# NikolasMarkou/blind_image_denoising

Measured on AMD Instinct MI355X. Metric: denoised images/sec (256x256x3) + MAE vs ref, resnet_1x18, higher is better.
Workload: dtype f16x2 split (hi+lo, fp32 accumulate)

## Files before the change

blind_image_denoising_amd/_native.py:

```python
import ctypes as C
import os
import pathlib

_HERE = pathlib.Path(__file__).resolve().parent
LIB_PATH = pathlib.Path(os.environ.get("BFCNN_HIP_LIB", _HERE / "lib" / "libbfcnn_hip.so"))

BF_OK, BF_EINVAL, BF_EUNSUPPORTED, BF_EWORKSPACE, BF_EHIP = 0, -1, -2, -3, -4
BF_ACT_LINEAR, BF_ACT_RELU, BF_ACT_LEAKY_RELU = 0, 1, 2
BF_REG_NONE, BF_REG_L1, BF_REG_L2 = 0, 1, 2
BF_MODE_INFERENCE, BF_MODE_TRAIN = 0, 1
BF_DTYPE_U8, BF_DTYPE_F32 = 0, 1
BF_LOSS_COUNT = 8
(BF_LOSS_TOTAL, BF_LOSS_DENOISER_TOTAL, BF_LOSS_MAE, BF_LOSS_MSE, BF_LOSS_SSIM,
 BF_LOSS_REGULARIZATION, BF_LOSS_MODEL_TOTAL, BF_LOSS_GRAD_NORM) = range(8)
EPI_RELU, EPI_AFFINE, EPI_RES, EPI_MASK, EPI_STATS, EPI_BNBWD = 1, 2, 4, 8, 16, 32


class ResnetDesc(C.Structure):
    _fields_ = [(n, C.c_int32) for n in (
        "struct_size", "in_channels", "filters", "kernel_size", "no_layers", "block_convs",
        "block_kernel", "activation", "base_activation", "use_bn", "head_filters",
        "head_activation", "out_channels", "denormalize", "reg_base", "reg_block", "reg_head")] + \
        [(n, C.c_float) for n in ("v_min", "v_max", "bn_eps", "bn_momentum", "leaky_alpha")]

# ... 135 lines not shown
    "bf_op_relu_shift_bwd": (_I, [_P, _I, _F, _P, _P, _I, _P]),
    "bf_op_normalize": (_I, [_P, _P, _I64, _F, _F, _I, _P]),
    "bf_op_channel_repeat": (_I, [_P, _P, _I64, _I, _I, _P]),
    "bf_op_channel_group_sum": (_I, [_P, _P, _I64, _I, _I, _P]),
    "bf_op_group_kernel": (_I, [_P, _P, _I, _I, _I, _I, _P]),
    "bf_op_flip_hw": (_I, [_P, _P, _I, _I, _P]),
    "bf_op_transpose2d": (_I, [_P, _P, _I, _I, _P]),
    "bf_comm_unique_id": (_I, [C.c_char_p]),
    "bf_comm_init_rank": (_I, [C.POINTER(_P), _I, _I, C.c_char_p]),
    "bf_comm_destroy": (_I, [_P]),
    "bf_allreduce_grads": (_I, [_P, _P, _I64, _P, _P]),
    "bf_comm_last_error": (C.c_char_p, []),
    "bf_op_channel_multiplier": (_I, [_P, _P, _I, _P]),
    "bf_op_prune_tensors": (_I, [_P, _I64, _P, _I, _I, _F, _F, _F, C.c_uint64, _P, _P, _P]),
    "bf_op_count_below": (_I, [_P, _I64, _P, _I, _F, _P, _P]),
    "bf_op_dihedral_stack_u8": (_I, [_P, _P, _P, _I, _I, _I, _I, _I, _P]),
    "bf_op_dihedral_merge": (_I, [_P, _P, _P, _I, _I, _I, _I, _I, _I, _P]),
    "bf_op_risk_probe_u8": (_I, [_P, _P, _I, _I, _I, _I, _I, _I, C.c_uint64, _P]),
    "bf_op_risk_sums_scratch_bytes": (_I64, [_I, _I, _I, _I, _I]),
    "bf_op_risk_sums": (_I, [_P, _P, _I, _I, _I, _I, _I, _I, C.c_uint64, _P, _I64, _P, _P]),
    "bf_op_risk_sums_affine_scratch_bytes": (_I64, [_I, _I, _I, _I, _I]),
    "bf_op_risk_sums_affine": (_I, [_P, _P, _I, _I, _I, _I, _I, _I, C.c_uint64, _P, _I64, _P, _P]),
    "bf_op_neighbor_pairs": (_I, [_P, _I, _P, _F, _P, _P, _I, _I, _I, _I, C.c_uint64, _P]),
    "bf_set_option": (_I, [_P, C.c_char_p, _I]),
    "bf_get_timing": (_I, [_P, C.POINTER(C.c_float), C.POINTER(C.c_int)]),
    "bf_get_block_kernel": (C.c_char_p, [_P, C.POINTER(C.c_int)]),
    "bf_get_train_kernels": (C.c_char_p, [_P]),
    "bf_debug_conv3x3": (_I, [_P, _P, _P, _P, _P, _P, _P, _P, _P, _I, _I, _I, _I, _I, _P]),
    "bf_debug_conv3x3_grid": (_I, [_I, _I, _I]),
    "bf_debug_h3_weight_scale": (_F, [_F]),
    "bf_debug_fused_block": (_I, [_P, _P, _P, _P, _P, _P, _P, _I, _I, _I, _I, _P]),
    "bf_debug_fused_block_h3_scratch_floats": (_I64, [_I, _I, _I]),
    "bf_debug_fused_block_h3": (_I, [_P, _P, _P, _P, _P, _P, _P, _I, _I, _I, _I, _P]),
    "bf_debug_fused_block2_h3_scratch_floats": (_I64, [_I, _I, _I]),
    "bf_debug_fused_block2_h3": (_I, [_P, _P, _P, _P, _P, _P, _I, _I, _I, _I, _I, _P]),
    "bf_debug_set_h3_variant": (_I, [_I]),
    "bf_debug_set_upsample_band": (_I, [_I]),
    "bf_debug_conv3x3_h3_scratch_floats": (_I64, []),
    "bf_debug_conv3x3_h3": (_I, [_P, _P, _P, _P, _P, _P, _P, _I, _I, _I, _I, _I, _P]),
    "bf_debug_wgrad_partial_floats": (_I64, [_I, _I, _I]),
    "bf_debug_wgrad3x3": (_I, [_P, _P, _P, _P, _I, _I, _I, _P]),
    "bf_debug_wgrad3x3_h3": (_I, [_P, _P, _P, _P, _I, _I, _I, _P]),
    "bf_debug_fwd_block_h3t_scratch_floats": (_I64, [_I, _I, _I]),
    "bf_debug_fwd_block_h3t": (_I, [_P, _P, _P, _P, _P, _P, _P, _P, _P, _P, _P, _I, _I, _I, _I, _I, _P]),
    "bf_debug_bwd_block_h3t_scratch_floats": (_I64, [_I, _I, _I]),
    "bf_debug_bwd_block_h3t": (_I, [_P, _P, _P, _P, _P, _P, _P, _P, _P, _P, _P, _P, _I, _I, _I, _I, _I, _P]),
    "bf_debug_conv3x3_h3_pre": (_I, [_P, _P, _P, _P, _P, _P, _P, _P, _I, _I, _I, _I, _I, _P]),
    "bf_debug_bwd3x3_h3_scratch_floats": (_I64, [_I, _I, _I]),
    "bf_debug_bwd3x3_h3_grid": (_I, [_I, _I, _I]),
    "bf_debug_bwd3x3_h3_grid_ex": (_I, [_I, _I, _I, _I]),
    "bf_debug_bwd3x3_h3": (_I, [_P, _P, _P, _P, _P, _P, _P, _P, _P, _P, _P, _I, _I, _I, _I, _I, _I, _P]),
    "bf_debug_forward_plan": (_I, [_P, _I, _I, _I, _I, C.c_char_p, _I]),
    "bf_debug_base_path": (_I, [_P, _I, _I, _I, _I, _I]),
    "bf_debug_mfma_probe": (_I, [_P, _P, _P, _P]),
}

BF_STATUS_BYTES = 2048
BF_STATUS_F16_RANGE = 1

_lib = None


class StreamArg(C.c_void_p):
    _bf_device = None


def _device_guard(fn):
    def call(*args):
        for a in args:
            dev = getattr(a, "_bf_device", None)
            if dev is not None:
                import torch
                if torch.cuda.current_device() != dev:
                    with torch.cuda.device(dev):
                        return fn(*args)
                break
        return fn(*args)
    call.raw = fn
    call.__name__ = getattr(fn, "__name__", "bf_call")
    return call


class _Library:

    def __init__(self, handle):
        self._handle = handle

    def __getattr__(self, name):
        return getattr(self._handle, name)


def lib():
    global _lib
    if _lib is None:
        if not LIB_PATH.exists():
            raise ImportError(
                f"{LIB_PATH} is missing: the gfx950 HIP library has not been built "
                f"(run blind_image_denoising_amd/csrc/build.sh). There is no CPU fallback.")
        handle = C.CDLL(str(LIB_PATH), mode=getattr(os, "RTLD_NOW", 2))
        wrapped = _Library(handle)
        for name, (res, args) in SIGNATURES.items():
            fn = getattr(handle, name)
            fn.restype = res
            fn.argtypes = args
            setattr(wrapped, name, _device_guard(fn))
        if handle.bf_abi_version() != 1:
# ... 53 lines not shown
```

blind_image_denoising_amd/csrc/bf_common.h:

```cpp
#pragma once
#include <hip/hip_runtime.h>
#include <stdint.h>
#include <stddef.h>
#include "../../include/bfcnn_hip.h"
#include "../../include/bfcnn_hip_debug.h"

typedef float f32x4 __attribute__((ext_vector_type(4)));

__device__ __forceinline__ f32x4 bf_acc_ready(f32x4 acc)
{
    asm volatile("s_nop 7" : "+v"(acc));
    return acc;
}


#include <mutex>
#include <unordered_set>
inline hipError_t bf_set_max_lds(const void* kernel, int bytes)
{
    static std::mutex mu;
    static std::unordered_set<uint64_t> done;
    int dev = 0;
    hipError_t e = hipGetDevice(&dev);
    if (e != hipSuccess) return e;
// ... 98 lines not shown
    int act1_relu;
    const void* zeros;
    void* dump;
    unsigned long long* dbg;
    const float* head_wh;
    void* head_out;
    int head_u8, Ho, Wo, denormalize;
    float v_min, v_max;
    int* status;
    int compact = 0;
};
struct H3Request {
    int B, H, W;
    int variant;
    bool head;
    bool compact;
};
enum class H3Kernel { Tiles32, Tiles16, FullRow };
struct H3Choice {
    H3Kernel kernel;
    bool bottom_up;
};
H3Choice   bf_select_fused_block_h3(const H3Request& r);
hipError_t bf_launch_fused_block_h3_as(const FusedH3Args& a, H3Kernel k, hipStream_t s);
hipError_t bf_launch_fused_block_h3(const FusedH3Args& a, hipStream_t s);
bool       bf_fused_block_h3_use_pairs(const H3Request& r);
const char* bf_fused_block_h3_kernel_name(H3Kernel k);
const char* bf_fused_block_kernel_name();
void       bf_set_h3_variant(int v);
hipError_t bf_launch_fused_block_h3v(const FusedH3Args& a, hipStream_t s);
bool       bf_fused_block_h3v_supports(int H, int W);
struct FusedH3WArgs {
    const void* in;
    void* out;
    const void* w1r[2];
    const void* w2r[2];
    const float* aux[2];
    int B, H, W;
    int nstrips, tiles_y, ntiles, rows_per_tile;
    int reverse_tiles;
    int act1_relu;
    const void* zeros;
    unsigned long long* dbg;
    const float* head_wh;
    void* head_out;
    int head_u8, Ho, Wo, denormalize;
    float v_min, v_max;
    int* status;
    const void* base_u8;
    const float* base_w;
    int Hs, Ws, base_relu;
};
hipError_t bf_launch_fused_block2_h3w(const FusedH3WArgs& a, hipStream_t s);
bool       bf_fused_block2_h3w_supports(int H, int W);
hipError_t bf_launch_pack_h3(const float* params, const float* state, int64_t p_blocks, int64_t p_stride, float* dst,
                             int64_t d_stride, int layers, int use_bn, float eps, const float* ext_scale,
                             const float* ext_shift, hipStream_t s);
#define BF_H3_TRAIN_PACK_FLOATS (BF_H3R_WPACK_FLOATS + 64)
#define BF_TRAIN_PACK_STRIDE BF_H3_TRAIN_PACK_FLOATS
hipError_t bf_launch_conv3x3_h3(const ConvArgs& a, int epi, hipStream_t s);
hipError_t bf_launch_wgrad3x3_h3(const float* x, const float* dy, float* partial, float* dw, int B, int H, int W, hipStream_t s);

struct BwdH3Args {
    const float* x;
    const float* g;
    const float* c;
    const float* coef;
    const float* wpack;
    float* out;
    const float* res;
    const float* bnc;
    float* wpartial;
    float* stats;
    int B, H, W, reverse;
    int reserved[4];
    int tiles_x, tiles_y, ntiles;
};
struct FwdBlockH3Args {
    const float* x;
    const float* pre_c;
    const float* pre_scale; const float* pre_shift;
    float* a_out;
    float* t_out;
    float* c_out;
    const float* wpack0;
    const float* wpack1;
    float* stats;
    int B, H, W, reverse, act_relu;
    int tiles_y, ntiles, rows_per_tile;
    const float* fin_partial;
    int fin_nblk;
    double fin_count;
    const float* fin_gamma;
    float *fin_mm, *fin_mv;
    float fin_eps, fin_momentum;
    float* fin_scale;
    float* fin_meaninv;
};
bool       bf_fwd_block_h3t_supports(int H, int W);
int        bf_fwd_block_h3t_grid(int B, int H, int W);
hipError_t bf_launch_fwd_block_h3t(const FwdBlockH3Args& a, hipStream_t s);
struct BwdBlockH3Args {
    const float* a;
    const float* g;
    const float* c;
    const float* coef;
// ... 106 lines not shown
```

blind_image_denoising_amd/csrc/debug_entry.hip:

```cpp
#include "bf_common.h"
#include "h3_weights.h"
#include <cstring>

extern "C" int bf_debug_conv3x3(const float* in, const float* w_hwio, float* out, const float* scale, const float* shift,
                                const float* res, const float* mask, float* stats, float* wpack_scratch, int B, int H, int W,
                                int epi, int transpose_flip, void* stream)
{
    hipStream_t s = (hipStream_t)stream;
    if (bf_launch_pack_conv(w_hwio, wpack_scratch, transpose_flip, s) != hipSuccess) return BF_EHIP;
    ConvArgs ca;
    memset(&ca, 0, sizeof(ca));
    ca.in = in; ca.out = out; ca.wpack = wpack_scratch; ca.scale = scale; ca.shift = shift; ca.res = res; ca.mask = mask;
    ca.stats = stats; ca.B = B; ca.H = H; ca.W = W;
    return bf_launch_conv3x3_c16(ca, epi, s) == hipSuccess ? BF_OK : BF_EHIP;
}

static unsigned long long* g_fused_dbg = nullptr;
extern "C" int bf_debug_set_fused_dbg(void* buf) { g_fused_dbg = (unsigned long long*)buf; return BF_OK; }

extern "C" int bf_debug_conv3x3_grid(int B, int H, int W) { return bf_conv3x3_c16_grid(B, H, W); }

extern "C" int bf_debug_fused_block(const float* in, const float* w1_hwio, const float* w2_hwio, const float* scale,
                                    const float* shift, float* out, float* wpack_scratch, int B, int H, int W, int act1_relu,
                                    void* stream)
// ... 30 lines not shown
    if (hipMemcpyAsync(params, w1_hwio, 2304 * 4, hipMemcpyDeviceToDevice, s) != hipSuccess) return BF_EHIP;
    if (hipMemcpyAsync(params + 2304, w2_hwio, 2304 * 4, hipMemcpyDeviceToDevice, s) != hipSuccess) return BF_EHIP;
    if (bf_launch_zero(zeros, 64, s) != hipSuccess) return BF_EHIP;
    if (bf_launch_pack_h3(params, state, 0, 4608 + 16, pk, BF_H3_BLOCK_FLOATS, 1, 0, 0.f, scale, shift, s) != hipSuccess) return BF_EHIP;
    if (bf_launch_h3_from_f32(in, xa, B, H, W, s) != hipSuccess) return BF_EHIP;
    FusedH3Args fa;
    fa.in = xa; fa.out = ya; fa.aux = pk;
    fa.w1r = fa.aux + 64; fa.w2r = fa.aux + 64 + BF_H3R_WPACK_FLOATS;
    fa.B = B; fa.H = H; fa.W = W; fa.tiles_x = fa.tiles_y = fa.ntiles = 0; fa.rows_per_tile = 0; fa.variant = -1; fa.reverse_tiles = 0; fa.act1_relu = act1_relu;
    fa.zeros = zeros; fa.dump = dump; fa.dbg = g_fused_dbg;
    fa.head_wh = nullptr; fa.head_out = nullptr; fa.head_u8 = 0; fa.Ho = fa.Wo = 0; fa.denormalize = 0; fa.v_min = fa.v_max = 0.f;
    fa.status = nullptr;
    if (bf_launch_fused_block_h3(fa, s) != hipSuccess) return BF_EHIP;
    return bf_launch_h3_to_f32(ya, out, B, H, W, s) == hipSuccess ? BF_OK : BF_EHIP;
}

extern "C" int64_t bf_debug_fused_block2_h3_scratch_floats(int B, int H, int W)
{
    return 2 * (int64_t)B * H * W * 16 + 2 * (int64_t)BF_H3_BLOCK_FLOATS + 2 * (4608 + 16) + 32 + 64;
}

extern "C" int bf_debug_fused_block2_h3(const float* in, const float* w_hwio, const float* scale, const float* shift, float* out,
                                        float* scratch, int B, int H, int W, int act1_relu, int reverse, void* stream)
{
    hipStream_t s = (hipStream_t)stream;
    if (!in || !w_hwio || !scale || !shift || !out || !scratch || B <= 0 || H <= 0 || W <= 0) return BF_EINVAL;
    const int64_t act = (int64_t)B * H * W * 16;
    float* xa = scratch;
    float* ya = scratch + act;
    float* pk = ya + act;
    float* params = pk + 2 * BF_H3_BLOCK_FLOATS;
    float* state = params + 2 * (4608 + 16);
    float* zeros = state + 32;
    if (hipMemcpyAsync(params, w_hwio, 4608 * 4, hipMemcpyDeviceToDevice, s) != hipSuccess) return BF_EHIP;
    if (hipMemcpyAsync(params + 4608 + 16, w_hwio + 4608, 4608 * 4, hipMemcpyDeviceToDevice, s) != hipSuccess) return BF_EHIP;
    if (bf_launch_zero(zeros, 64, s) != hipSuccess) return BF_EHIP;
    for (int b = 0; b < 2; ++b)
        if (bf_launch_pack_h3(params + b * (4608 + 16), state, 0, 4608 + 16, pk + b * BF_H3_BLOCK_FLOATS, BF_H3_BLOCK_FLOATS, 1, 0,
                              0.f, scale + 16 * b, shift + 16 * b, s) != hipSuccess) return BF_EHIP;
    if (bf_launch_h3_from_f32(in, xa, B, H, W, s) != hipSuccess) return BF_EHIP;
    FusedH3WArgs fa;
    memset(&fa, 0, sizeof(fa));
    fa.in = xa; fa.out = ya;
    for (int b = 0; b < 2; ++b) {
        const float* aux = pk + b * BF_H3_BLOCK_FLOATS;
        fa.aux[b] = aux; fa.w1r[b] = aux + 64; fa.w2r[b] = aux + 64 + BF_H3R_WPACK_FLOATS;
    }
    fa.B = B; fa.H = H; fa.W = W; fa.reverse_tiles = reverse ? 1 : 0; fa.act1_relu = act1_relu;
    fa.zeros = zeros; fa.dbg = g_fused_dbg;
    if (bf_launch_fused_block2_h3w(fa, s) != hipSuccess) return BF_EHIP;
    return bf_launch_h3_to_f32(ya, out, B, H, W, s) == hipSuccess ? BF_OK : BF_EHIP;
}

extern "C" int bf_debug_set_h3_variant(int variant)
{
    bf_set_h3_variant(variant);
    return BF_OK;
}

extern "C" int64_t bf_debug_conv3x3_h3_scratch_floats(void) { return 4 * (int64_t)BF_H3_TRAIN_PACK_FLOATS + 2 * 2304 + 16; }
extern "C" int bf_debug_conv3x3_h3(const float* in, const float* w_hwio, float* out, const float* res, const float* mask,
                                   float* stats, float* scratch, int B, int H, int W, int epi, int transpose_flip, void* stream)
{
    hipStream_t s = (hipStream_t)stream;
    float* params = scratch + 4 * BF_H3_TRAIN_PACK_FLOATS;
    if (hipMemcpyAsync(params, w_hwio, 2304 * 4, hipMemcpyDeviceToDevice, s) != hipSuccess) return BF_EHIP;
    if (hipMemcpyAsync(params + 2304, w_hwio, 2304 * 4, hipMemcpyDeviceToDevice, s) != hipSuccess) return BF_EHIP;
    if (bf_launch_pack_h3_train(params, 0, 4608 + 16, scratch, 1, 2, 2320, s) != hipSuccess) return BF_EHIP;
    ConvArgs ca;
    memset(&ca, 0, sizeof(ca));
    ca.in = in; ca.out = out; ca.wpack = scratch + (transpose_flip ? 2 : 0) * BF_H3_TRAIN_PACK_FLOATS;
    ca.res = res; ca.mask = mask; ca.stats = stats; ca.B = B; ca.H = H; ca.W = W;
    return bf_launch_conv3x3_h3(ca, epi, s) == hipSuccess ? BF_OK : BF_EHIP;
}

extern "C" int bf_debug_conv3x3_h3_pre(const float* in, const float* pre_c, const float* pre_scale, const float* pre_shift,
                                       float* pre_out, const float* w_hwio, float* out, float* scratch, int B, int H, int W, int relu,
                                       int reverse, void* stream)
{
    hipStream_t s = (hipStream_t)stream;
    float* params = scratch + 4 * BF_H3_TRAIN_PACK_FLOATS;
    if (hipMemcpyAsync(params, w_hwio, 2304 * 4, hipMemcpyDeviceToDevice, s) != hipSuccess) return BF_EHIP;
    if (hipMemcpyAsync(params + 2304, w_hwio, 2304 * 4, hipMemcpyDeviceToDevice, s) != hipSuccess) return BF_EHIP;
    if (bf_launch_pack_h3_train(params, 0, 4608 + 16, scratch, 1, 2, 2320, s) != hipSuccess) return BF_EHIP;
    ConvArgs ca;
    memset(&ca, 0, sizeof(ca));
    ca.in = in; ca.out = out; ca.wpack = scratch; ca.B = B; ca.H = H; ca.W = W; ca.reverse = reverse;
    ca.pre_c = pre_c; ca.pre_scale = pre_scale; ca.pre_shift = pre_shift; ca.pre_out = pre_out;
    return bf_launch_conv3x3_h3(ca, relu ? EPI_RELU : 0, s) == hipSuccess ? BF_OK : BF_EHIP;
}

extern "C" int64_t bf_debug_fwd_block_h3t_scratch_floats(int B, int H, int W)
{
    return 4 * (int64_t)BF_H3_TRAIN_PACK_FLOATS + 2 * 2304 + 16 + (int64_t)bf_fwd_block_h3t_grid(B, H, W) * 32;
}
extern "C" int bf_debug_fwd_block_h3t(const float* x, const float* pre_c, const float* pre_scale, const float* pre_shift,
                                      const float* w0_hwio, const float* w1_hwio, float* a_out, float* t_out, float* c_out, float* stats,
                                      float* scratch, int B, int H, int W, int relu, int reverse, void* stream)
{
    hipStream_t s = (hipStream_t)stream;
    if (!bf_fwd_block_h3t_supports(H, W)) return BF_EUNSUPPORTED;
    float* params = scratch + 4 * BF_H3_TRAIN_PACK_FLOATS;
    if (hipMemcpyAsync(params, w0_hwio, 2304 * 4, hipMemcpyDeviceToDevice, s) != hipSuccess) return BF_EHIP;
    if (hipMemcpyAsync(params + 2304, w1_hwio, 2304 * 4, hipMemcpyDeviceToDevice, s) != hipSuccess) return BF_EHIP;
    if (bf_launch_pack_h3_train(params, 0, 4608 + 16, scratch, 1, 2, 2320, s) != hipSuccess) return BF_EHIP;
    float* partial = params + 2 * 2304 + 16;
// ... 106 lines not shown
```

blind_image_denoising_amd/csrc/fused_h3w.hip:

```cpp
#include "h3v_core.h"
#include "h3_bands.h"
#include "base_rows.h"

#ifndef H3W_PRIO_SET
#define H3W_PRIO_SET 0
#endif
#if H3W_PRIO_SET == 1
#define H3W_PRIO_A1 0
#define H3W_PRIO_B1 1
#define H3W_PRIO_A2 2
#define H3W_PRIO_B2 3
#elif H3W_PRIO_SET == 2
#define H3W_PRIO_A1 3
#define H3W_PRIO_B1 2
#define H3W_PRIO_A2 1
#define H3W_PRIO_B2 0
#elif H3W_PRIO_SET == 3
#define H3W_PRIO_A1 0
#define H3W_PRIO_B1 2
#define H3W_PRIO_A2 0
#define H3W_PRIO_B2 2
#elif H3W_PRIO_SET == 4
#define H3W_PRIO_A1 2
#define H3W_PRIO_B1 0
// ... 511 lines not shown
        char* orow = reinterpret_cast<char*>(a.head_out) + ((size_t)t.b * a.Ho + (size_t)t.y(k)) * a.Wo * 3 * (a.head_u8 ? 1 : 4);
        const char* src = tout + oslot * Gm::OUT_SLOT + st_off;
        float h0 = 0.f, h1 = 0.f, h2 = 0.f;
#pragma unroll
        for (int hf = 0; hf < 2; ++hf) {
            const h8 hi = *reinterpret_cast<const h8*>(src + hf * Gm::OUT_PLANE), lo = *reinterpret_cast<const h8*>(src + (2 + hf) * Gm::OUT_PLANE);
#pragma unroll
            for (int c = 0; c < 8; ++c) {
                const float v = (float)hi[c] + (float)lo[c];
                const f32x4 w = *reinterpret_cast<const f32x4*>(a.head_wh + (hf * 8 + c) * 4);
                h0 = fmaf(v, w.x, h0);
                h1 = fmaf(v, w.y, h1);
                h2 = fmaf(v, w.z, h2);
            }
        }
        const bool finite = fabsf(h0) <= 3.0e38f && fabsf(h1) <= 3.0e38f && fabsf(h2) <= 3.0e38f;
        if (!finite && a.status) atomicOr(a.status, BF_STATUS_F16_RANGE);
        float r[3] = {h0, h1, h2};
#pragma unroll
        for (int o = 0; o < 3; ++o) {
            float v = (1.0f - 2.0f / (__expf(4.0f * r[o]) + 1.0f)) * 0.51f;
            if (a.denormalize) v = (fminf(fmaxf(v, -0.5f), 0.5f) + 0.5f) * (a.v_max - a.v_min) + a.v_min;
            r[o] = v;
        }
        if (!okc) return;
        if (a.head_u8) {
            unsigned char* p = reinterpret_cast<unsigned char*>(orow) + (size_t)col * 3;
#pragma unroll
            for (int o = 0; o < 3; ++o) p[o] = (unsigned char)fminf(fmaxf(rintf(r[o]), 0.f), 255.f);
        } else {
            float* p = reinterpret_cast<float*>(orow) + (size_t)col * 3;
#pragma unroll
            for (int o = 0; o < 3; ++o) p[o] = r[o];
        }
        __builtin_amdgcn_sched_barrier(0);
    }
    __device__ __forceinline__ void after_first_group() {}
    __device__ __forceinline__ void end() {}
    __device__ __forceinline__ void finish() {}
};

#ifndef H3W_BASE_SPREAD
#define H3W_BASE_SPREAD 1
#endif
constexpr int h3w_base_groups(const int role)
{
    return H3W_BASE_SPREAD == 0 ? (role == 2 ? 3 : 0) : (H3W_BASE_SPREAD == 1 ? (role >= 1 ? 1 : 0) : (role <= 2 ? 1 : 0));
}
constexpr int h3w_base_first_group(const int role, const int rw)
{
    return H3W_BASE_SPREAD == 0 ? 3 * rw : (H3W_BASE_SPREAD == 1 ? 3 * (role - 1) + rw : 3 * role + rw);
}
constexpr bool h3w_base_fetches(const int role) { return role == 2; }

template <int NGW, bool FETCH>
struct H3WProducer {
    using Gm = H3WGeom;
    const FusedH3WArgs& a;
    char* tx0;
    char* tring;
    const char* twa;
    int g0, fw;
    float inv_s, floor_;
    int wr;
    int fo;
    int col0;
    int px, xcol;
    const uint8_t* img;
    unsigned raw[3];
    BrPixel rawp;
    int dslot;

    __device__ __forceinline__ H3WProducer(const FusedH3WArgs& a_, char* lds, const int g0_, const int fw_)
        : a(a_), tx0(lds + Gm::X0_OFF), tring(lds + Gm::BIN_OFF), twa(lds + Gm::BWA_OFF), g0(g0_), fw(fw_), wr(0), fo(0), col0(0),
          px(0), xcol(0), img(nullptr), raw{0u, 0u, 0u}, rawp{false, false}, dslot(0)
    {
        inv_s = *reinterpret_cast<const float*>(lds + Gm::BINVS_OFF);
        floor_ = a.base_relu ? 0.f : -__builtin_inff();
    }
    __device__ __forceinline__ void set_tile(const H3WTile& t, const int lane)
    {
        const int n = lane & 15, q = lane >> 4, gc0 = 16 * g0 + n;
        wr = (q >> 1) * Gm::X0_PLANE + (gc0 + 1) * 16 + (q & 1) * 8;
        const int p = gc0 + 2 * (q & 1);
        fo = ((p & 1) * Gm::BIN_ROWPX + (p & ~1)) * 8;
        twa = tx0 - Gm::X0_OFF + Gm::BWA_OFF + lane * 16;
        col0 = t.G0 + gc0;
        px = 64 * fw + lane;
        xcol = t.G0 - 1 + px;
        img = reinterpret_cast<const uint8_t*>(a.base_u8) + (size_t)t.b * a.Hs * a.Ws * 3;
    }
    __device__ __forceinline__ void request(const H3WTile& t, const int u)
    {
        const int yy = t.ybase + u - 5;
        const bool need = (px < Gm::GW + 2) & (u <= t.nrows + 9);
        rawp = br_pixel(yy, xcol, a.H, a.W, a.Hs, a.Ws);
        rawp.inside &= need;
        rawp.colour &= need;
        if (rawp.colour) {
            const uint8_t* p = img + ((size_t)yy * a.Ws + xcol) * 3;
            raw[0] = p[0];
            raw[1] = p[1];
            raw[2] = p[2];
        }
    }
    __device__ __forceinline__ void commit(const int u)
    {
        if (px >= Gm::GW + 2) return;
        const h4 v = br_record(rawp, raw[0], raw[1], raw[2]);
        h4* row = reinterpret_cast<h4*>(tring + (u & (Gm::BIN_RING - 1)) * Gm::BIN_SLOT);
        row[px] = v;
        if (px > 0) row[Gm::BIN_ROWPX + px - 1] = v;
    }
    __device__ __forceinline__ void produce(const H3WTile& t, const int r, const int slot)
    {
        if (r >= t.nrows + 8) return;
        const int y = t.y(r - 4);
        const bool rowok = (y >= 0) & (y < a.H);
        f32x4 acc[NGW];
#pragma unroll
        for (int g = 0; g < NGW; ++g) acc[g] = (f32x4){0.f, 0.f, 0.f, 0.f};
#pragma unroll
        for (int dy = 0; dy < 3; ++dy) {
            const h8 wa = *reinterpret_cast<const h8*>(twa + dy * 64 * 16);
            const char* row = tring + ((r + dy) & (Gm::BIN_RING - 1)) * Gm::BIN_SLOT + fo;
#pragma unroll
            for (int g = 0; g < NGW; ++g) acc[g] = MFMA_H(wa, *reinterpret_cast<const h8*>(row + g * 128), acc[g]);
        }
#pragma unroll
        for (int g = 0; g < NGW; ++g) {
            H3VEpi<true> e;
            e.v = bf_acc_ready(acc[g]);
            e.sc = (rowok & (col0 + 16 * g < a.W)) ? inv_s : 0.f;
            e.floor_ = floor_;
            e.p = tx0 + wr + slot * Gm::PITCH + g * 256;
            e.lo_off = 2 * Gm::X0_PLANE;
            e.all();
        }
    }
    __device__ __forceinline__ void fill(const H3WTile& t)
    {
        if constexpr (FETCH) {
#pragma unroll
            for (int u = 0; u < Gm::BIN_RING; ++u) {
                request(t, u);
                commit(u);
            }
            request(t, Gm::BIN_RING);
        }
    }
    __device__ __forceinline__ void prologue(const H3WTile& t)
    {
        produce(t, 0, 0);
        dslot = 1;
    }
    __device__ __forceinline__ void begin(const H3WTile& t, const int s)
    {
        if constexpr (FETCH) {
            commit(s + 4);
            request(t, s + 5);
        }
        produce(t, s + 1, dslot);
        dslot = h3v_wrap(dslot + 1, Gm::NRX0);
        __builtin_amdgcn_sched_barrier(0);
    }
};

template <>
struct H3WProducer<0, false> {
    __device__ __forceinline__ H3WProducer(const FusedH3WArgs&, char*, int, int) {}
    __device__ __forceinline__ void set_tile(const H3WTile&, int) {}
    __device__ __forceinline__ void fill(const H3WTile&) {}
    __device__ __forceinline__ void prologue(const H3WTile&) {}
    __device__ __forceinline__ void begin(const H3WTile&, int) {}
};

template <bool HEAD>
constexpr bool h3w_direct() { return H3W_DIRECT_STORE != 0 && !HEAD; }
template <bool HEAD, bool BASE>
constexpr int h3w_hook_kind(const int role)
{
    const int k = h3w_mem_kind(role);
    return k == 2 ? (HEAD ? 3 : (h3w_direct<HEAD>() ? 0 : 2)) : ((BASE && k == 1) ? 0 : k);
}

template <bool HEAD, bool BASE>
__global__ __launch_bounds__(H3WGeom::NT, 3) void fused_block2_h3w_kernel(FusedH3WArgs a)
{
    using Gm = H3WGeom;
    extern __shared__ __attribute__((aligned(16))) char h3w_lds[];
    char* tx0 = h3w_lds + Gm::X0_OFF;
    char* tm1 = h3w_lds + Gm::M1_OFF;
    char* tx1 = h3w_lds + Gm::X1_OFF;
    char* tm2 = h3w_lds + Gm::M2_OFF;
    constexpr bool DIRECT = h3w_direct<HEAD>();
    constexpr int LDS_RINGS = DIRECT ? Gm::LDS_BYTES : Gm::LDS_BYTES_STAGED;
    char* tout = DIRECT ? nullptr : h3w_lds + Gm::OUT_OFF;
    const int tid = threadIdx.x, lane = tid & 63;
    const int wave = __builtin_amdgcn_readfirstlane(tid >> 6);
    const int n = lane & 15;
    const int role = wave / Gm::NR, rw = wave - role * Gm::NR;
    const unsigned plane_g = (unsigned)a.H * (unsigned)a.W * 16u;
    const int gc0 = 16 * Gm::G * rw + n;

    if (BASE && a.status && blockIdx.x == 0 && tid == 0) *a.status = 0;
    for (int i = tid * 16; i < (BASE ? Gm::LDS_BYTES_BASE : LDS_RINGS); i += Gm::NT * 16)
        *reinterpret_cast<f32x4*>(h3w_lds + i) = (f32x4){0.f, 0.f, 0.f, 0.f};
    __syncthreads();
    if constexpr (BASE) {
        const float bs = br_weight_scale(a.base_w, reinterpret_cast<float*>(h3w_lds + Gm::BRED_OFF));
        if (wave == 0) {
#pragma unroll
            for (int dy = 0; dy < 3; ++dy)
                *reinterpret_cast<h8*>(h3w_lds + Gm::BWA_OFF + (dy * 64 + lane) * 16) = br_operand(a.base_w, bs, dy, lane);
            if (lane == 0) *reinterpret_cast<float*>(h3w_lds + Gm::BINVS_OFF) = 1.0f / bs;
        }
        __syncthreads();
    }

#if H3V_ABLATE & 32
    unsigned long long stamp_sum[Gm::NSTAMP] = {0, 0, 0, 0}, stamp_prev, real0;
    asm volatile("s_memrealtime %0\n\ts_memtime %1\n\ts_waitcnt lgkmcnt(0)" : "=s"(real0), "=s"(stamp_prev)::"memory");
#endif

#define H3W_ROW_IN_IMAGE(k) ((t.y(k) >= 0) & (t.y(k) < a.H))
#define H3W_BAND(R, M, P, ACTIVE, STEP)                                                                         \
    for (int ti = blockIdx.x; ti < a.ntiles; ti += gridDim.x) {                                               \
        const H3WTile t = h3w_tile(a, ti);                                                                    \
        R.set_tile(t, a.W, gc0);                                                                              \
        M.set_tile(t, lane);                                                                                  \
        P.set_tile(t, lane);                                                                                  \
        if constexpr (BASE) {                                      \
            P.fill(t);                                                                                        \
            h3v_barrier();                                                                                    \
        }                                                                                                     \
        P.prologue(t);                                                                                        \
        M.prologue(t);                                                                                        \
        h3v_barrier();                                                 \
        const int nsteps = t.nrows + Gm::LEAD;                                                                \
        int slot5 = 0;                                                                           \
        for (int s0 = 0; s0 < nsteps; s0 += Gm::UNROLL) {                                                     \
            H3W_ONE(0, M, P, ACTIVE, STEP); H3W_ONE(1, M, P, ACTIVE, STEP); H3W_ONE(2, M, P, ACTIVE, STEP);   \
            H3W_ONE(3, M, P, ACTIVE, STEP); H3W_ONE(4, M, P, ACTIVE, STEP); H3W_ONE(5, M, P, ACTIVE, STEP);   \
        }                                                                                                     \
        M.finish();                                                                                           \
        h3v_barrier();                                                                                        \
    }
#define H3W_ONE(PH, M, P, ACTIVE, STEP)                                                                         \
    do {                                                                                                      \
        const int s = s0 + PH;                                                                                \
        P.begin(t, s);                                                                                        \
        M.begin(t, s, PH);                                                                                    \
        if (ACTIVE(s)) { STEP(PH); }                                                                          \
        else M.after_first_group();                                                                           \
        slot5 = h3v_wrap(slot5 + 1, Gm::NRX0);                                                                \
        H3V_STAMP(0);                                                                                         \
        M.end();                                                                                              \
        H3V_STAMP(1);                                                                                         \
        h3v_barrier();                                                                                        \
        H3V_STAMP(2);                                                                                         \
    } while (0)

    if (role == 0) {
        __builtin_amdgcn_s_setprio(H3W_PRIO_A1);
        H3WRoleA<Gm::X0_PLANE> R;
        R.tin = tx0; R.tmid = tm1;
        R.init(a.w1r[0], a, a.aux[0], lane, gc0);
        R.skip_last = (H3V_ABLATE & 256) && rw == Gm::NR - 1;
        H3WMem<h3w_hook_kind<HEAD, BASE>(0)> M(a, tx0, tout, rw, plane_g);
        H3WProducer<BASE ? h3w_base_groups(0) : 0, BASE && h3w_base_groups(0) && h3w_base_fetches(0)> P(a, h3w_lds, h3w_base_first_group(0, rw), rw);
        __builtin_amdgcn_s_waitcnt(h3_vmcnt(0));
#define H3W_ACTIVE(s) ((s) < t.nrows + 8)
#define H3W_STEP(PH) R.template step<PH>(slot5 * Gm::PITCH, (s >= 2) & H3W_ROW_IN_IMAGE(s - 5), M)
        H3W_BAND(R, M, P, H3W_ACTIVE, H3W_STEP)
#undef H3W_ACTIVE
#undef H3W_STEP
    } else if (role == 1) {
        __builtin_amdgcn_s_setprio(H3W_PRIO_B1);
        H3WRoleB<Gm::X0_PLANE, Gm::X1_PLANE> R;
        R.tmid = tm1; R.tres = tx0; R.tout = tx1;
        R.init(a.w2r[0], a, a.aux[0], lane, gc0, true);
        R.skip_last = (H3V_ABLATE & 256) && rw == Gm::NR - 1;
        H3WMem<h3w_hook_kind<HEAD, BASE>(1)> M(a, tx0, tout, rw, plane_g);
        H3WProducer<BASE ? h3w_base_groups(1) : 0, BASE && h3w_base_groups(1) && h3w_base_fetches(1)> P(a, h3w_lds, h3w_base_first_group(1, rw), rw);
        __builtin_amdgcn_s_waitcnt(h3_vmcnt(0));
#define H3W_ACTIVE(s) (((s) >= 3) & ((s) < t.nrows + 9))
#define H3W_STEP(PH) R.template step<PH>(h3v_wrap(slot5 + Gm::NRX0 - 1, Gm::NRX0) * Gm::PITCH, (PH % Gm::NRX1) * Gm::PITCH, H3W_ROW_IN_IMAGE(s - 7), M)
        H3W_BAND(R, M, P, H3W_ACTIVE, H3W_STEP)
#undef H3W_ACTIVE
#undef H3W_STEP
    } else if (role == 2) {
        __builtin_amdgcn_s_setprio(H3W_PRIO_A2);
        H3WRoleA<Gm::X1_PLANE> R;
        R.tin = tx1; R.tmid = tm2;
        R.init(a.w1r[1], a, a.aux[1], lane, gc0);
        R.skip_last = (H3V_ABLATE & 256) && rw == Gm::NR - 1;
        H3WMem<h3w_hook_kind<HEAD, BASE>(2)> M(a, tx0, tout, rw, plane_g);
        H3WProducer<BASE ? h3w_base_groups(2) : 0, BASE && h3w_base_groups(2) && h3w_base_fetches(2)> P(a, h3w_lds, h3w_base_first_group(2, rw), rw);
        __builtin_amdgcn_s_waitcnt(h3_vmcnt(0));
#define H3W_ACTIVE(s) (((s) >= 6) & ((s) < t.nrows + 10))
#define H3W_STEP(PH) R.template step<PH>(((PH + 2) % Gm::NRX1) * Gm::PITCH, H3W_ROW_IN_IMAGE(s - 9), M)
        H3W_BAND(R, M, P, H3W_ACTIVE, H3W_STEP)
#undef H3W_ACTIVE
#undef H3W_STEP
    } else {
        __builtin_amdgcn_s_setprio(H3W_PRIO_B2);
        H3WRoleB<Gm::X1_PLANE, Gm::OUT_PLANE, DIRECT> R;
        R.tmid = tm2; R.tres = tx1; R.tout = tout;
        R.init(a.w2r[1], a, a.aux[1], lane, gc0, false);
        R.skip_last = (H3V_ABLATE & 256) && rw == Gm::NR - 1;
        H3WMem<h3w_hook_kind<HEAD, BASE>(3)> M(a, tx0, tout, rw, plane_g);
        H3WProducer<BASE ? h3w_base_groups(3) : 0, BASE && h3w_base_groups(3) && h3w_base_fetches(3)> P(a, h3w_lds, h3w_base_first_group(3, rw), rw);
        __builtin_amdgcn_s_waitcnt(h3_vmcnt(0));
#define H3W_ACTIVE(s) (((s) >= 9) & ((s) < t.nrows + 11))
#define H3W_STEP(PH) R.set_row(t, a.W, s - (Gm::LEAD - 1)); R.template step<PH>(((PH + 1) % Gm::NRX1) * Gm::PITCH, (PH % Gm::NRO) * Gm::OUT_SLOT, true, M)
        H3W_BAND(R, M, P, H3W_ACTIVE, H3W_STEP)
#undef H3W_ACTIVE
#undef H3W_STEP
    }
#undef H3W_BAND
#undef H3W_ONE
#undef H3W_ROW_IN_IMAGE
#if H3V_ABLATE & 32
    {
        unsigned long long real1;
        asm volatile("s_memrealtime %0\n\ts_waitcnt lgkmcnt(0)" : "=s"(real1)::"memory");
        stamp_sum[3] = real1 - real0;
    }
    if (a.dbg && lane == 0) {
        for (int k = 0; k < Gm::NSTAMP; ++k) a.dbg[((size_t)blockIdx.x * Gm::NW + wave) * 8 + k] = stamp_sum[k];
    }
#endif
}

bool bf_fused_block2_h3w_supports(int H, int W) { return W >= 1 && H >= 1; }

hipError_t bf_launch_fused_block2_h3w(const FusedH3WArgs& args, hipStream_t s)
{
    using Gm = H3WGeom;
    FusedH3WArgs a = args;
    if (!a.zeros || (!a.in && !a.base_u8) || (!a.out && !a.head_wh) || !bf_fused_block2_h3w_supports(a.H, a.W)) return hipErrorInvalidValue;
    if (a.base_u8 && (!a.base_w || a.head_wh || a.reverse_tiles || a.Hs < 1 || a.Ws < 1 || a.Hs > a.H || a.Ws > a.W)) return hipErrorInvalidValue;
    if ((int64_t)a.H * a.W * 64 >= ((int64_t)1 << 32)) return hipErrorInvalidValue;
    const BandPlan p = bf_band_plan(a.B, a.H, (a.W + Gm::SW - 1) / Gm::SW, Gm::LEAD + 2);
    a.nstrips = p.nstrips;
    a.rows_per_tile = p.rows_per_tile;
    a.tiles_y = p.tiles_y;
    a.ntiles = p.ntiles;
    if (a.head_wh && (!a.head_out || a.Ho < 1 || a.Wo < 1 || a.Ho > a.H || a.Wo > a.W)) return hipErrorInvalidValue;
    void (*kernel)(FusedH3WArgs) = a.base_u8 ? fused_block2_h3w_kernel<false, true>
                                   : a.head_wh ? fused_block2_h3w_kernel<true, false> : fused_block2_h3w_kernel<false, false>;
    const int lds = a.base_u8 ? Gm::LDS_BYTES_BASE : (a.head_wh ? Gm::LDS_BYTES_STAGED : Gm::LDS_BYTES);
    const hipError_t e = bf_set_max_lds(reinterpret_cast<const void*>(kernel), lds);
    if (e != hipSuccess) return e;
    hipLaunchKernelGGL(kernel, dim3(p.grid), dim3(Gm::NT), lds, s, a);
    return hipGetLastError();
}
```

include/bfcnn_hip_debug.h:

```cpp
#ifndef BFCNN_HIP_DEBUG_H
#define BFCNN_HIP_DEBUG_H
#include "bfcnn_hip.h"
#ifdef __cplusplus
extern "C" {
#endif

int bf_debug_conv3x3(const float* in, const float* w_hwio, float* out, const float* scale, const float* shift,
                     const float* res, const float* mask, float* stats, float* wpack_scratch,
                     int batch, int height, int width, int epi, int transpose_flip, void* stream);
int bf_debug_conv3x3_grid(int batch, int height, int width);
int bf_debug_fused_block(const float* in, const float* w1_hwio, const float* w2_hwio, const float* scale,
                         const float* shift, float* out, float* wpack_scratch,
                         int batch, int height, int width, int act1_relu, void* stream);
int64_t bf_debug_fused_block_h3_scratch_floats(int batch, int height, int width);
int bf_debug_fused_block_h3(const float* in, const float* w1_hwio, const float* w2_hwio, const float* scale,
                            const float* shift, float* out, float* scratch,
                            int batch, int height, int width, int act1_relu, void* stream);
int64_t bf_debug_fused_block2_h3_scratch_floats(int batch, int height, int width);
int bf_debug_fused_block2_h3(const float* in, const float* w_hwio, const float* scale, const float* shift, float* out,
                             float* scratch, int batch, int height, int width, int act1_relu, int reverse, void* stream);
int bf_debug_set_h3_variant(int variant);
int64_t bf_debug_conv3x3_h3_scratch_floats(void);
int bf_debug_conv3x3_h3(const float* in, const float* w_hwio, float* out, const float* res, const float* mask, float* stats,
                        float* scratch, int batch, int height, int width, int epi, int transpose_flip, void* stream);
int64_t bf_debug_wgrad_partial_floats(int batch, int height, int width);
int bf_debug_wgrad3x3(const float* x, const float* dy, float* partial, float* dw,
                      int batch, int height, int width, void* stream);
int bf_debug_wgrad3x3_h3(const float* x, const float* dy, float* partial, float* dw,
                         int batch, int height, int width, void* stream);
int bf_debug_conv3x3_h3_pre(const float* in, const float* pre_c, const float* pre_scale, const float* pre_shift, float* pre_out,
                            const float* w_hwio, float* out, float* scratch, int batch, int height, int width, int relu,
                            int reverse, void* stream);
int64_t bf_debug_fwd_block_h3t_scratch_floats(int batch, int height, int width);
int bf_debug_fwd_block_h3t(const float* x, const float* pre_c, const float* pre_scale, const float* pre_shift, const float* w0_hwio,
                           const float* w1_hwio, float* a_out, float* t_out, float* c_out, float* stats, float* scratch, int batch,
                           int height, int width, int relu, int reverse, void* stream);
int64_t bf_debug_bwd_block_h3t_scratch_floats(int batch, int height, int width);
int bf_debug_bwd_block_h3t(const float* a, const float* g, const float* c, const float* coef, const float* w0_hwio, const float* w1_hwio,
                           const float* bnc, float* out, float* dw1, float* dw0, float* stats, float* scratch, int batch, int height,
                           int width, int relu, int reverse, void* stream);
int64_t bf_debug_bwd3x3_h3_scratch_floats(int batch, int height, int width);
int bf_debug_bwd3x3_h3_grid(int batch, int height, int width);
int bf_debug_bwd3x3_h3_grid_ex(int batch, int height, int width, int dbuf);
int bf_debug_bwd3x3_h3(const float* x, const float* g, const float* c, const float* coef, const float* w_hwio, float* out,
                       const float* res, const float* bnc, float* dw, float* stats, float* scratch, int batch, int height,
                       int width, int epi, int reverse, int repack, void* stream);
int bf_debug_forward_plan(bf_handle h, int batch, int height, int width, int pad_pow2, char* out, int out_bytes);
int bf_debug_base_path(bf_handle h, int batch, int height, int width, int pad_pow2, int in_is_u8);
float bf_debug_h3_weight_scale(float max_abs);
int bf_debug_mfma_probe(const float* a, const float* b, float* d, void* stream);
int bf_debug_set_upsample_band(int on);

#ifdef __cplusplus
}
#endif
#endif
```

Baseline: 31230.

## Roll base-conv producer accumulators across rows to reuse each input fragment

The base-conv producer in the fused block kernel now keeps three rolling accumulators per column group. Each new input row fragment is loaded once and fed to all three vertical taps, where before every output row reloaded three input rows from the LDS ring. A prime step seeds the accumulators, and weights can optionally stay in registers. The ReLU floor was dropped from the producer epilogue, and the launch check now rejects base_relu, so that case is no longer supported. This costs extra VGPRs for the persistent accumulators, which may reduce occupancy.

```diff
diff --git a/blind_image_denoising_amd/_native.py b/blind_image_denoising_amd/_native.py
--- a/blind_image_denoising_amd/_native.py
+++ b/blind_image_denoising_amd/_native.py
@@ -211,6 +211,7 @@
     "bf_debug_bwd3x3_h3": (_I, [_P, _P, _P, _P, _P, _P, _P, _P, _P, _P, _P, _I, _I, _I, _I, _I, _I, _P]),
     "bf_debug_forward_plan": (_I, [_P, _I, _I, _I, _I, C.c_char_p, _I]),
     "bf_debug_base_path": (_I, [_P, _I, _I, _I, _I, _I]),
+    "bf_debug_pair_launch_check": (_I, [_I, _I]),
     "bf_debug_mfma_probe": (_I, [_P, _P, _P, _P]),
 }
 
diff --git a/blind_image_denoising_amd/csrc/bf_common.h b/blind_image_denoising_amd/csrc/bf_common.h
--- a/blind_image_denoising_amd/csrc/bf_common.h
+++ b/blind_image_denoising_amd/csrc/bf_common.h
@@ -174,6 +174,7 @@
     int Hs, Ws, base_relu;
 };
 hipError_t bf_launch_fused_block2_h3w(const FusedH3WArgs& a, hipStream_t s);
+hipError_t bf_fused_block2_h3w_check(const FusedH3WArgs& a);
 bool       bf_fused_block2_h3w_supports(int H, int W);
 hipError_t bf_launch_pack_h3(const float* params, const float* state, int64_t p_blocks, int64_t p_stride, float* dst,
                              int64_t d_stride, int layers, int use_bn, float eps, const float* ext_scale,
diff --git a/blind_image_denoising_amd/csrc/debug_entry.hip b/blind_image_denoising_amd/csrc/debug_entry.hip
--- a/blind_image_denoising_amd/csrc/debug_entry.hip
+++ b/blind_image_denoising_amd/csrc/debug_entry.hip
@@ -106,6 +106,23 @@
     return bf_launch_h3_to_f32(ya, out, B, H, W, s) == hipSuccess ? BF_OK : BF_EHIP;
 }
 
+extern "C" int bf_debug_pair_launch_check(int producer, int base_relu)
+{
+    static const float placeholder[16] = {0.f};
+    FusedH3WArgs fa;
+    memset(&fa, 0, sizeof(fa));
+    fa.out = const_cast<float*>(placeholder);
+    fa.zeros = placeholder;
+    fa.B = 2; fa.H = 64; fa.W = 64;
+    if (producer) {
+        fa.base_u8 = placeholder; fa.base_w = placeholder; fa.Hs = 64; fa.Ws = 64;
+    } else {
+        fa.in = placeholder;
+    }
+    fa.base_relu = base_relu;
+    return bf_fused_block2_h3w_check(fa) == hipSuccess ? BF_OK : BF_EINVAL;
+}
+
 extern "C" int bf_debug_set_h3_variant(int variant)
 {
     bf_set_h3_variant(variant);
diff --git a/blind_image_denoising_amd/csrc/fused_h3w.hip b/blind_image_denoising_amd/csrc/fused_h3w.hip
--- a/blind_image_denoising_amd/csrc/fused_h3w.hip
+++ b/blind_image_denoising_amd/csrc/fused_h3w.hip
@@ -587,6 +587,12 @@
     return H3W_BASE_SPREAD == 0 ? 3 * rw : (H3W_BASE_SPREAD == 1 ? 3 * (role - 1) + rw : 3 * role + rw);
 }
 constexpr bool h3w_base_fetches(const int role) { return role == 2; }
+#ifndef H3W_BASE_ROLL
+#define H3W_BASE_ROLL 1
+#endif
+#ifndef H3W_BASE_WA_REG
+#define H3W_BASE_WA_REG 0
+#endif
 
 template <int NGW, bool FETCH>
 struct H3WProducer {
@@ -596,7 +602,9 @@
     char* tring;
     const char* twa;
     int g0, fw;
-    float inv_s, floor_;
+    float inv_s;
+    h8 wa[3];
+    f32x4 acc[NGW][3];
     int wr;
     int fo;
     int col0;
@@ -611,7 +619,28 @@
           px(0), xcol(0), img(nullptr), raw{0u, 0u, 0u}, rawp{false, false}, dslot(0)
     {
         inv_s = *reinterpret_cast<const float*>(lds + Gm::BINVS_OFF);
-        floor_ = a.base_relu ? 0.f : -__builtin_inff();
+        if constexpr (H3W_BASE_WA_REG) {
+#pragma unroll
+            for (int dy = 0; dy < 3; ++dy) wa[dy] = *reinterpret_cast<const h8*>(lds + Gm::BWA_OFF + (dy * 64 + (threadIdx.x & 63)) * 16);
+        }
+    }
+    __device__ __forceinline__ h8 operand(const int dy) const
+    {
+        if constexpr (H3W_BASE_WA_REG) return wa[dy];
+        else return *reinterpret_cast<const h8*>(twa + dy * 64 * 16);
+    }
+    __device__ __forceinline__ void epilogue(const int g, const int slot, const f32x4 v, const bool rowok) const
+    {
+        H3VEpi<false> e;
+        e.v = v;
+        e.sc = (rowok & (col0 + 16 * g < a.W)) ? inv_s : 0.f;
+        e.p = tx0 + wr + slot * Gm::PITCH + g * 256;
+        e.lo_off = 2 * Gm::X0_PLANE;
+        e.all();
+    }
+    __device__ __forceinline__ h8 fragment(const int u, const int g) const
+    {
+        return *reinterpret_cast<const h8*>(tring + (u & (Gm::BIN_RING - 1)) * Gm::BIN_SLOT + fo + g * 128);
     }
     __device__ __forceinline__ void set_tile(const H3WTile& t, const int lane)
     {
@@ -652,26 +681,57 @@
         if (r >= t.nrows + 8) return;
         const int y = t.y(r - 4);
         const bool rowok = (y >= 0) & (y < a.H);
-        f32x4 acc[NGW];
-#pragma unroll
-        for (int g = 0; g < NGW; ++g) acc[g] = (f32x4){0.f, 0.f, 0.f, 0.f};
+        f32x4 c[NGW];
+#pragma unroll
+        for (int g = 0; g < NGW; ++g) c[g] = (f32x4){0.f, 0.f, 0.f, 0.f};
 #pragma unroll
         for (int dy = 0; dy < 3; ++dy) {
-            const h8 wa = *reinterpret_cast<const h8*>(twa + dy * 64 * 16);
-            const char* row = tring + ((r + dy) & (Gm::BIN_RING - 1)) * Gm::BIN_SLOT + fo;
-#pragma unroll
-            for (int g = 0; g < NGW; ++g) acc[g] = MFMA_H(wa, *reinterpret_cast<const h8*>(row + g * 128), acc[g]);
-        }
+            const h8 w = operand(dy);
+#pragma unroll
+            for (int g = 0; g < NGW; ++g) c[g] = MFMA_H(w, fragment(r + dy, g), c[g]);
+        }
+#pragma unroll
+        for (int g = 0; g < NGW; ++g) epilogue(g, slot, bf_acc_ready(c[g]), rowok);
+    }
+    template <int PH>
+    __device__ __forceinline__ void roll(const H3WTile& t, const int s, const int slot)
+    {
+        const int r = s + 1;
+        if (r >= t.nrows + 8) return;
+        constexpr int a_done = (PH + 1) % 3, a_mid = (PH + 2) % 3, a_new = PH % 3;
+        const int y = t.y(r - 4);
+        const bool rowok = (y >= 0) & (y < a.H);
+        h8 b[NGW];
+#pragma unroll
+        for (int g = 0; g < NGW; ++g) b[g] = fragment(s + 3, g);
+        const h8 w2 = operand(2), w1 = operand(1), w0 = operand(0);
+#pragma unroll
+        for (int g = 0; g < NGW; ++g) acc[g][a_done] = MFMA_H(w2, b[g], acc[g][a_done]);
+        __builtin_amdgcn_sched_barrier(0);
+#pragma unroll
+        for (int g = 0; g < NGW; ++g) acc[g][a_mid] = MFMA_H(w1, b[g], acc[g][a_mid]);
+        __builtin_amdgcn_sched_barrier(0);
+#pragma unroll
+        for (int g = 0; g < NGW; ++g) acc[g][a_new] = MFMA_H(w0, b[g], ((f32x4){0.f, 0.f, 0.f, 0.f}));
+        __builtin_amdgcn_sched_barrier(0);
+#pragma unroll
+        for (int g = 0; g < NGW; ++g) epilogue(g, slot, acc[g][a_done], rowok);
+    }
+    __device__ __forceinline__ void prime(const H3WTile& t)
+    {
+        const int y = t.y(-4);
+        const bool rowok = (y >= 0) & (y < a.H);
+        const h8 w0 = operand(0), w1 = operand(1), w2 = operand(2);
 #pragma unroll
         for (int g = 0; g < NGW; ++g) {
-            H3VEpi<true> e;
-            e.v = bf_acc_ready(acc[g]);
-            e.sc = (rowok & (col0 + 16 * g < a.W)) ? inv_s : 0.f;
-            e.floor_ = floor_;
-            e.p = tx0 + wr + slot * Gm::PITCH + g * 256;
-            e.lo_off = 2 * Gm::X0_PLANE;
-            e.all();
-        }
+            const h8 b0 = fragment(0, g), b1 = fragment(1, g), b2 = fragment(2, g);
+            const f32x4 zero = {0.f, 0.f, 0.f, 0.f};
+            acc[g][0] = MFMA_H(w2, b2, MFMA_H(w1, b1, MFMA_H(w0, b0, zero)));
+            acc[g][1] = MFMA_H(w1, b2, MFMA_H(w0, b1, zero));
+            acc[g][2] = MFMA_H(w0, b2, zero);
+        }
+#pragma unroll
+        for (int g = 0; g < NGW; ++g) epilogue(g, 0, bf_acc_ready(acc[g][0]), rowok);
     }
     __device__ __forceinline__ void fill(const H3WTile& t)
     {
@@ -686,16 +746,19 @@
     }
     __device__ __forceinline__ void prologue(const H3WTile& t)
     {
-        produce(t, 0, 0);
+        if constexpr (H3W_BASE_ROLL) prime(t);
+        else produce(t, 0, 0);
         dslot = 1;
     }
+    template <int PH>
     __device__ __forceinline__ void begin(const H3WTile& t, const int s)
     {
         if constexpr (FETCH) {
             commit(s + 4);
             request(t, s + 5);
         }
-        produce(t, s + 1, dslot);
+        if constexpr (H3W_BASE_ROLL) roll<PH>(t, s, dslot);
+        else produce(t, s + 1, dslot);
         dslot = h3v_wrap(dslot + 1, Gm::NRX0);
         __builtin_amdgcn_sched_barrier(0);
     }
@@ -707,7 +770,7 @@
     __device__ __forceinline__ void set_tile(const H3WTile&, int) {}
     __device__ __forceinline__ void fill(const H3WTile&) {}
     __device__ __forceinline__ void prologue(const H3WTile&) {}
-    __device__ __forceinline__ void begin(const H3WTile&, int) {}
+    template <int PH> __device__ __forceinline__ void begin(const H3WTile&, int) {}
 };
 
 template <bool HEAD>
@@ -784,7 +847,7 @@
 #define H3W_ONE(PH, M, P, ACTIVE, STEP)                                                                         \
     do {                                                                                                      \
         const int s = s0 + PH;                                                                                \
-        P.begin(t, s);                                                                                        \
+        P.template begin<PH>(t, s);                                                                           \
         M.begin(t, s, PH);                                                                                    \
         if (ACTIVE(s)) { STEP(PH); }                                                                          \
         else M.after_first_group();                                                                           \
@@ -870,19 +933,26 @@
 
 bool bf_fused_block2_h3w_supports(int H, int W) { return W >= 1 && H >= 1; }
 
+hipError_t bf_fused_block2_h3w_check(const FusedH3WArgs& a)
+{
+    if (!a.zeros || (!a.in && !a.base_u8) || (!a.out && !a.head_wh) || !bf_fused_block2_h3w_supports(a.H, a.W)) return hipErrorInvalidValue;
+    if (a.base_u8 && (!a.base_w || a.head_wh || a.reverse_tiles || a.Hs < 1 || a.Ws < 1 || a.Hs > a.H || a.Ws > a.W || a.base_relu)) return hipErrorInvalidValue;
+    if ((int64_t)a.H * a.W * 64 >= ((int64_t)1 << 32)) return hipErrorInvalidValue;
+    if (a.head_wh && (!a.head_out || a.Ho < 1 || a.Wo < 1 || a.Ho > a.H || a.Wo > a.W)) return hipErrorInvalidValue;
+    return hipSuccess;
+}
+
 hipError_t bf_launch_fused_block2_h3w(const FusedH3WArgs& args, hipStream_t s)
 {
     using Gm = H3WGeom;
     FusedH3WArgs a = args;
-    if (!a.zeros || (!a.in && !a.base_u8) || (!a.out && !a.head_wh) || !bf_fused_block2_h3w_supports(a.H, a.W)) return hipErrorInvalidValue;
-    if (a.base_u8 && (!a.base_w || a.head_wh || a.reverse_tiles || a.Hs < 1 || a.Ws < 1 || a.Hs > a.H || a.Ws > a.W)) return hipErrorInvalidValue;
-    if ((int64_t)a.H * a.W * 64 >= ((int64_t)1 << 32)) return hipErrorInvalidValue;
+    const hipError_t bad = bf_fused_block2_h3w_check(a);
+    if (bad != hipSuccess) return bad;
     const BandPlan p = bf_band_plan(a.B, a.H, (a.W + Gm::SW - 1) / Gm::SW, Gm::LEAD + 2);
     a.nstrips = p.nstrips;
     a.rows_per_tile = p.rows_per_tile;
     a.tiles_y = p.tiles_y;
     a.ntiles = p.ntiles;
-    if (a.head_wh && (!a.head_out || a.Ho < 1 || a.Wo < 1 || a.Ho > a.H || a.Wo > a.W)) return hipErrorInvalidValue;
     void (*kernel)(FusedH3WArgs) = a.base_u8 ? fused_block2_h3w_kernel<false, true>
                                    : a.head_wh ? fused_block2_h3w_kernel<true, false> : fused_block2_h3w_kernel<false, false>;
     const int lds = a.base_u8 ? Gm::LDS_BYTES_BASE : (a.head_wh ? Gm::LDS_BYTES_STAGED : Gm::LDS_BYTES);
diff --git a/include/bfcnn_hip_debug.h b/include/bfcnn_hip_debug.h
--- a/include/bfcnn_hip_debug.h
+++ b/include/bfcnn_hip_debug.h
@@ -19,6 +19,7 @@
 int64_t bf_debug_fused_block2_h3_scratch_floats(int batch, int height, int width);
 int bf_debug_fused_block2_h3(const float* in, const float* w_hwio, const float* scale, const float* shift, float* out,
                              float* scratch, int batch, int height, int width, int act1_relu, int reverse, void* stream);
+int bf_debug_pair_launch_check(int producer, int base_relu);
 int bf_debug_set_h3_variant(int variant);
 int64_t bf_debug_conv3x3_h3_scratch_floats(void);
 int bf_debug_conv3x3_h3(const float* in, const float* w_hwio, float* out, const float* res, const float* mask, float* stats,
```

New measurement: 31420 (median of 6 runs). No clear change (+0.6%).
